# bcgsc/abyss

Hardware: AMD Instinct MI355X
Metric: Mk-mers/s inserted+extended (abyss-bloom-dbg, k=64); unitig bit-exact (higher is better)
Workload: dtype u64

## Files before the change

abyss_amd/_lib.py:

```python
from __future__ import annotations

import ctypes as C
import os

from . import build

ABG_OK = 0
ABG_EINVAL, ABG_ENODEV, ABG_ENOMEM, ABG_EINTERNAL, ABG_EAGAIN = -1, -2, -3, -4, -5


class Params(C.Structure):
    _fields_ = [
        ("k", C.c_uint32), ("num_hashes", C.c_uint32), ("min_cov", C.c_uint32), ("trim", C.c_uint32),
        ("bloom_bytes", C.c_uint64), ("counters", C.c_uint64), ("spaced_seed", C.c_char_p),
        ("device", C.c_int32), ("verbose", C.c_int32), ("insert_batch_kmers", C.c_uint64),
        ("claim_log2", C.c_uint32), ("walk_slots", C.c_uint32), ("wtab_log2", C.c_uint32),
        ("cascade_levels", C.c_uint32), ("slice_filter", C.c_uint32), ("reserved_", C.c_uint32 * 5),
    ]


class Counters(C.Structure):
    _fields_ = [(n, C.c_uint64) for n in
                ("solid_reads", "visited_reads", "reads_processed", "bases_assembled", "next_contig_id")]


class Contig(C.Structure):
    _fields_ = [
        ("contig_id", C.c_uint64), ("read_index", C.c_uint64), ("seq", C.c_char_p),
        ("length", C.c_uint32), ("coverage", C.c_uint32), ("redundant", C.c_int32),
        ("left_ext", C.c_uint32), ("right_ext", C.c_uint32), ("left_code", C.c_int32),
        ("right_code", C.c_int32), ("seed_pos", C.c_uint32),
    ]


class Stats(C.Structure):
    _fields_ = [(n, C.c_uint64) for n in
                ("insert_rounds", "walk_rounds", "candidates", "walked", "rewalked", "commit_breaks",
                 "commit_rounds", "generated", "bulk_calls", "bulk_steps", "lin_steps", "guide_slots", "chain_steps", "batch_cuts", "overflows", "memo_hits", "memo_adds", "tiled_ops", "tiled_pending", "tile_overflows", "cls_covered_reads", "archive_bases", "cls_decided_reads", "counter_bytes_held",
                 "commit_rounds_incremental", "commit_dirty_records", "commit_first_chunk_decided")]


CONTIG_CB = C.CFUNCTYPE(None, C.c_void_p, C.POINTER(Contig))
TEXT_CB = C.CFUNCTYPE(None, C.c_void_p, C.POINTER(C.c_char), C.c_uint64)

_lib = None


def symbols():
    return [
        "abg_params_init", "abg_create", "abg_destroy", "abg_last_error", "abg_reset", "abg_filter_size",
        "abg_load_seqs", "abg_load_seqs_v", "abg_keep_reads", "abg_assemble_kept", "abg_load_packed", "abg_counting_stats", "abg_counters_export",
        "abg_counters_import", "abg_visited_export", "abg_visited_import", "abg_assemble_seqs", "abg_assemble_seqs_v",
        "abg_assemble_packed", "abg_cascade_export", "abg_get_counters", "abg_set_counters", "abg_hash_seq",
        "abg_contains_seq",
        "abg_attach_comm", "abg_share_reads", "abg_rccl_unique_id", "abg_rccl_comm_create", "abg_rccl_comm_destroy",
        "abg_dev_copy", "abg_dev_alloc", "abg_dev_free", "abg_output_graph_seqs",
        "abg_profile_enable", "abg_profile_reset", "abg_profile_get", "abg_get_stats",
        "abg_overlap_create", "abg_overlap_destroy", "abg_overlap_last_error", "abg_overlap_join", "abg_overlap_edges",
        "abg_overlap_profile", "abg_overlap_profile_get",
        "abg_rr_create", "abg_rr_destroy", "abg_rr_last_error", "abg_rr_bytes", "abg_rr_clear", "abg_rr_insert_seqs",
        "abg_rr_contains_seqs", "abg_rr_popcount", "abg_rr_export", "abg_rr_sync", "abg_rr_profile", "abg_rr_profile_get",
        "abg_kn_create", "abg_kn_destroy", "abg_kn_last_error", "abg_kn_import", "abg_kn_export", "abg_kn_insert_seqs",
        "abg_kn_contains_seqs", "abg_kn_popcount", "abg_kn_hash_seq", "abg_kn_sync", "abg_kn_profile", "abg_kn_profile_get",
        "abg_fm_create", "abg_fm_destroy", "abg_fm_last_error", "abg_fm_build", "abg_fm_size", "abg_fm_export", "abg_fm_map_seqs",
        "abg_fm_sync", "abg_fm_tune", "abg_fm_profile", "abg_fm_profile_get",
    ]


def load(path: str | None = None):
    global _lib
    if _lib is not None:
        return _lib
# ... 99 lines not shown
```

abyss_amd/csrc/abg_core.h:

```cpp
#pragma once

#include <stdint.h>
#include <stddef.h>

#if defined(__HIPCC__)
#include <hip/hip_runtime.h>
#define ABG_HD __host__ __device__ __forceinline__
#define ABG_HDN __host__ __device__
#define ABG_HDX __host__ __device__ __attribute__((noinline))
#else
#define ABG_HD inline
#define ABG_HDN
#define ABG_HDX
#endif

namespace abg {

constexpr int MAX_NW = 6;
constexpr int MAX_HASHES = 32;
constexpr unsigned FP_TRIM = 5;

enum Dir : int { FORWARD = 0, REVERSE = 1 };
enum Sense : int { SENSE = 0, ANTISENSE = 1 };

// ... 1141 lines not shown
{
	if (!coop) return atomic_min_u32(p, v);
	uint32_t r = 0;
	if (__lane_id() == 0) r = atomic_min_u32(p, v);
	return (uint32_t)__builtin_amdgcn_readfirstlane((int)r);
}
ABG_HD uint32_t wu_atomic_add_u32(uint32_t* p, uint32_t v, bool coop)
{
	if (!coop) return atomic_add_u32(p, v);
	uint32_t r = 0;
	if (__lane_id() == 0) r = atomic_add_u32(p, v);
	return (uint32_t)__builtin_amdgcn_readfirstlane((int)r);
}
ABG_HD uint64_t wu_atomic_add_u64(uint64_t* p, uint64_t v, bool coop)
{
	if (!coop) return atomic_add_u64(p, v);
	uint64_t r = 0;
	if (__lane_id() == 0) r = atomic_add_u64(p, v);
	return ((uint64_t)(uint32_t)__builtin_amdgcn_readfirstlane((int)(r >> 32)) << 32) |
	       (uint32_t)__builtin_amdgcn_readfirstlane((int)(uint32_t)r);
}
ABG_HD void wu_st_coherent(uint64_t* p, uint64_t v, bool coop)
{
	if (!coop || __lane_id() == 0) st_coherent(p, v);
}
ABG_HD void wu_st_u32(uint32_t* p, uint32_t v, bool coop)
{
	if (!coop || __lane_id() == 0) *p = v;
}
ABG_HD void wu_st_u8(uint8_t* p, uint8_t v, bool coop)
{
	if (!coop || __lane_id() == 0) *p = v;
}
#else
ABG_HD void wu_st_coherent(uint64_t* p, uint64_t v, bool) { st_coherent(p, v); }
ABG_HD void wu_st_u32(uint32_t* p, uint32_t v, bool) { *p = v; }
ABG_HD void wu_st_u8(uint8_t* p, uint8_t v, bool) { *p = v; }
ABG_HD uint64_t wu_cas_u64(uint64_t* p, uint64_t e, uint64_t v, bool) { return cas_u64(p, e, v); }
ABG_HD uint32_t wu_atomic_min_u32(uint32_t* p, uint32_t v, bool) { return atomic_min_u32(p, v); }
ABG_HD uint32_t wu_atomic_add_u32(uint32_t* p, uint32_t v, bool) { return atomic_add_u32(p, v); }
ABG_HD uint64_t wu_atomic_add_u64(uint64_t* p, uint64_t v, bool) { return atomic_add_u64(p, v); }
#endif

struct Guide {
	const uint64_t* tab;
	uint64_t mask;
	const uint32_t* words;
	uint64_t nwords;
	uint8_t* seen;
};
constexpr unsigned SV_VALID = 0x80u, SV_SIMPLE = 0x01u;
constexpr uint32_t GUIDE_MAX_NK = 256;
ABG_HD uint64_t guide_slot(uint64_t hm, uint64_t mask)
{
	uint64_t x = hm * 0x9E3779B97F4A7C15ULL;
	x ^= x >> 29;
	return x & mask;
}
ABG_HD uint32_t guide_tag(uint64_t hm) { return (uint32_t)(hm >> 56); }
ABG_HD uint64_t guide_pack(uint64_t woff, uint32_t pos, uint32_t nk, uint32_t tag)
{
	return (1ULL << 63) | ((uint64_t)(tag & 0xFFu) << 55) | ((uint64_t)(nk - 1) << 47) | ((uint64_t)pos << 39) | woff;
}
constexpr uint64_t GUIDE_MAX_WOFF = (1ULL << 39) - 1;
constexpr uint32_t BULK_LANES = 64, BULK_MIN = 4;
struct BulkScratch {
	VKey key[BULK_LANES];
	uint8_t good[BULK_LANES];
	uint8_t fbase[BULK_LANES];
	uint32_t dup[2 * BULK_LANES];
	uint32_t dupstop;
	uint32_t full;
	uint64_t hw[MAX_NW], hfh, hrh, hdf, hdr;
	struct Chain { uint64_t w[MAX_NW], fh, rh, df, dr; uint32_t depth, state; } chain[4];
};
enum { CB_ACTIVE = 0,
       CB_TRUE = 1,
       CB_NOT_CHAIN = 2,
       CB_NONE = 3,
       CB_FALSE = 4 };
enum { WSTAT_BULK_CALLS = 0, WSTAT_BULK_STEPS, WSTAT_LIN_STEPS, WSTAT_CHAIN_STEPS, WSTAT_MEMO_HITS, WSTAT_MEMO_ADDS,
       WSTAT_OVF_POOL, WSTAT_OVF_RECS,
       WSTAT_CLS_COVERED,
       WSTAT_CLS_DECIDED,
       WSTAT_N = 16 };

struct SuccMemo {
	uint64_t* k0;
	uint64_t* k1;
	uint64_t* val;
	uint64_t mask;
};
constexpr uint64_t MEMO_EMPTY = ~0ULL;
constexpr unsigned MEMO_PROBES = 8;
ABG_HD uint64_t memo_slot(const SuccMemo& m, uint64_t fh, uint64_t rh, int dir)
{
	uint64_t x = (fh ^ (rh * 0x9E3779B97F4A7C15ULL)) + (uint64_t)dir;
	x ^= x >> 31; x *= 0xD6E8FEB86659FD93ULL; x ^= x >> 29;
	return x & m.mask;
}
ABG_HD int memo_find(const SuccMemo& m, uint64_t fh, uint64_t rh, int dir)
{
	if (fh == MEMO_EMPTY || rh == MEMO_EMPTY) return -1;
	uint64_t s = memo_slot(m, fh, rh, dir);
	for (unsigned i = 0; i < MEMO_PROBES; i++, s = (s + 1) & m.mask) {
		const uint64_t a = ld_coherent(&m.k0[s]);
		if (a == MEMO_EMPTY) return -1;
		if (a != fh) continue;
		const uint64_t v = ld_coherent(&m.val[s]);
		if (!(v >> 63) || (int)((v >> 8) & 1u) != dir) continue;
		if (ld_coherent(&m.k1[s]) != rh) continue;
		return (int)(v & 0xFFu);
	}
	return -1;
}
ABG_HD void memo_add(const SuccMemo& m, uint64_t fh, uint64_t rh, int dir, unsigned code, unsigned base, bool coop)
{
// ... 895 lines not shown
```

abyss_amd/csrc/abg_engine.h:

```cpp
#pragma once
#include "abg_walk.h"

#include <algorithm>
#include <chrono>
#include <cstdio>
#include <cstdlib>
#include <cstring>
#include <functional>
#include <future>
#include <string>
#include <type_traits>
#include <vector>

namespace abg {

struct Failure { int code; std::string msg; };
constexpr int FAIL_INVAL = -1, FAIL_NOMEM = -3, FAIL_INTERNAL = -4;
[[noreturn]] inline void fail_now(int code, const std::string& msg) { throw Failure{ code, msg }; }
inline std::string strf(const char* fmt, unsigned long long a = 0, unsigned long long b = 0)
{
	char buf[256];
	snprintf(buf, sizeof buf, fmt, a, b);
	return buf;
}
// ... 17 lines not shown
	bool cosettle = true;
	uint32_t cosettle_passes = 6;
	uint32_t cosettle_log2 = 24;
	uint32_t walk_slots = 4096;
	uint32_t tb_cap = 512;
	uint32_t buf_cap = 1u << 16;
	uint64_t pool_cap = 1ull << 28;
	uint32_t rec_cap = 1u << 22;
	uint32_t wtab_log2 = 26;
	uint32_t wtab_log2_max = 31;
	uint32_t cend_log2 = 20;
	uint64_t p2_first_batch = 65536;
	uint64_t p2_max_batch = 1ull << 22;
	uint32_t p2_growth = 2;
	uint32_t p2_crowded = 1u << 18;
	uint32_t p2_starved_growth = 2;
	uint32_t p2_starved = 6144;
	uint32_t slice_filter = 0;
	bool solid_plane = true;
	uint32_t classify_slots = 65536;
	uint32_t cls_both_max_mb = 1024;
	bool cls_both = true;
	bool prefetch_classify = true;
	uint32_t memo_log2 = 0;
	bool memo = true;
	uint32_t p2_max_candidates = 1u << 18;
	uint32_t t_tags = 1024;
	uint32_t commit_incremental = 1;
	uint32_t commit_dirty_max = 4096;
	uint32_t commit_dirty_log2 = 26;
	uint32_t guide_stride = 4;
	uint32_t guide_log2_max = 31;
	bool guide_seen = true;
	bool link_duplicates = true;
	bool par_commit = true;
	bool overlap_bins = true;
	bool overlap_purity = true;
	uint32_t dist_hash_all_ranks = 2;
	uint32_t dist_route_min_ranks = 4;
	uint64_t keep_insert_scratch_bytes = 16ull << 30;
	uint64_t par_commit_max_bytes = 16ull << 30;
	int verbose = 0;
};

struct Counters {
	uint64_t solid_reads = 0, visited_reads = 0, reads_processed = 0, bases_assembled = 0,
	         contig_id = 0;
};

struct BaseCodes {
	uint8_t t[256];
	BaseCodes()
	{
		for (int i = 0; i < 256; i++) t[i] = 0xFF;
		t['A'] = t['a'] = 0; t['C'] = t['c'] = 1; t['G'] = t['g'] = 2; t['T'] = t['t'] = 3;
	}
};
template <class T>
struct NoInitAlloc : std::allocator<T> {
	template <class U> struct rebind { using other = NoInitAlloc<U>; };
	template <class U, class... A> void construct(U* p, A&&... a)
	{
		if constexpr (sizeof...(A) == 0) ::new ((void*)p) U; else ::new ((void*)p) U(std::forward<A>(a)...);
	}
};
struct HostBatch {
// ... 3183 lines not shown
			if (guide_tab_) be_.free(guide_tab_);
			guide_tab_ = (uint64_t*)be_.try_alloc(8ull << log2);
			guide_log2_ = log2;
			if (!guide_tab_) { if (cfg_.verbose) fprintf(stderr, "abyss_amd: no memory for the walkers' guide table, walking step by step\n"); return; }
		}
		be_.memset(guide_tab_, 0, 8ull << log2);
		guide_.mask = (1ull << log2) - 1; guide_.words = b.words; guide_.nwords = nwords;
		dispatch_nw([&](auto nw) {
			FGuideBuild<decltype(nw)::value> f{ p2_, b, cnt2_, guide_tab_, guide_.mask, cfg_.guide_stride, sampled };
			be_.launch_wave((sampled + GUIDE_READS_PER_ITEM - 1) / GUIDE_READS_PER_ITEM, f, "guide_build");
		});
		guide_.tab = guide_tab_;
		guide_slots_ = guide_.mask + 1;
		if (cfg_.guide_seen) {
			const uint64_t need = nwords * 16, total = be_.device_mem_bytes();
			if (guide_seen_ && guide_seen_bytes_ < need) { be_.free(guide_seen_); guide_seen_ = nullptr; }
			if (!guide_seen_ && (!total || need <= total / 24)) { guide_seen_ = (uint8_t*)be_.try_alloc(need); guide_seen_bytes_ = need; }
			if (guide_seen_) { be_.memset(guide_seen_, 0, need); guide_.seen = guide_seen_; }
		}
	}
	uint64_t next_batch_size() const
	{
		if (last_candidates_ > cfg_.p2_crowded) return std::max<uint64_t>(p2_batch_ / 2, 1024);
		if (last_candidates_ < cfg_.p2_starved) return std::min<uint64_t>(p2_batch_ * cfg_.p2_starved_growth, 8 * cfg_.p2_max_batch);
		return std::min<uint64_t>(p2_batch_ * cfg_.p2_growth, cfg_.p2_max_batch);
	}
	void clear_wstats()
	{
		be_.memset(wstats_, 0, WSTAT_N * 8);
	}
	struct Stats { uint64_t rounds = 0, walked = 0, rewalked = 0, candidates = 0, breaks = 0, insert_rounds = 0, commit_rounds = 0, generated = 0;
	               uint64_t bulk_calls = 0, bulk_steps = 0, lin_steps = 0, guide_slots = 0, chain_steps = 0, batch_cuts = 0, overflows = 0, memo_hits = 0, memo_adds = 0;
	               uint64_t tiled_ops = 0, tiled_pending = 0, tile_overflows = 0, cls_covered_reads = 0, archive_bases = 0, cls_decided_reads = 0;
	               uint64_t commit_rounds_incremental = 0, commit_dirty_records = 0, commit_first_chunk_decided = 0; };
	Stats stats()
	{
		Stats s = stats_;
		if (wstats_) {
			uint64_t v[WSTAT_N];
			be_.d2h(v, wstats_, sizeof v);
			s.bulk_calls = v[WSTAT_BULK_CALLS]; s.bulk_steps = v[WSTAT_BULK_STEPS]; s.lin_steps = v[WSTAT_LIN_STEPS]; s.chain_steps = v[WSTAT_CHAIN_STEPS];
			s.memo_hits = v[WSTAT_MEMO_HITS]; s.memo_adds = v[WSTAT_MEMO_ADDS];
			s.cls_covered_reads = v[WSTAT_CLS_COVERED]; s.cls_decided_reads = v[WSTAT_CLS_DECIDED];
		}
		if (arc_.seq && arc_valid_) { uint64_t u = 0; be_.d2h(&u, arc_.used, 8); s.archive_bases = std::min(u, arc_.cap) - ARC_HEAD; }
		s.guide_slots = guide_slots_;
		return s;
	}

  private:
	BE& be_;
	Config cfg_;
	Params p_;
	uint64_t m_ = 0, vis_bytes_ = 0;
	uint8_t* cnt_ = nullptr;
	uint8_t* vis_ = nullptr;
	CommitState* cstate_ = nullptr;
	uint64_t* scal_ = nullptr;
	Cascade casc_{ nullptr, 0, 0 };
	MaskTab* mask_d_ = nullptr;
	std::chrono::steady_clock::time_point dbg_t0_;
	uint32_t* T_ = nullptr;
	uint32_t t_tag_ = 0;
	uint64_t* Tk_ = nullptr; uint32_t* Tv_ = nullptr; uint32_t Tlog2_ = 0;
	uint64_t T_entries_ = 0;
	uint32_t* pcA_ = nullptr; uint64_t pcA_bits_ = 0; uint32_t pcA_shift_ = 0;
	bool t_hashed() const { return t_force_hashed_ || m_ * 4ull > cfg_.par_commit_max_bytes; }
	bool t_force_hashed_ = false;
	bool use_par_commit()
	{
		if (!cfg_.par_commit || t_failed_) return false;
		if (t_hashed()) return true;
		if (!T_) {
			T_ = (uint32_t*)be_.try_alloc(m_ * 4ull);
			t_tag_ = 0;
			if (!T_ && sliced_) {
// ... 746 lines not shown
		walk_ready_ = false;
	}
	void grow_walk_resources()
	{
		free_walk_scratch();
		walk_tb_cap_ *= 4;
		walk_buf_cap_ *= 8;
		if (walk_buf_cap_ > (1u << 28) || wtab_log2_ > 31) {
			fail_now(FAIL_INTERNAL, "a unitig exceeds the walker limits");
		}
		while ((uint64_t)wslots_ * walk_buf_cap_ > (8ull << 30) && wslots_ > 64) wslots_ /= 2;
		alloc_walk_scratch();
		free_tab(wtab_);
		wtab_log2_++;
		alloc_tab(wtab_, wtab_log2_);
		be_.free(pool_); be_.free(kh_);
		pool_cap_ *= 2;
		pool_ = (uint8_t*)be_.alloc(pool_cap_);
		kh_ = (uint64_t*)be_.alloc(pool_cap_ * 8);
		if (cfg_.verbose)
			fprintf(stderr, "abyss_amd: walker resources grown: %u frames, %u bases, 2^%u table, %llu pool\n",
			    walk_tb_cap_, walk_buf_cap_, wtab_log2_, (unsigned long long)pool_cap_);
	}

	template <int NW>
	WalkEnv<NW> make_env(const Batch& b, uint32_t* cand_d, uint32_t* status_d, uint32_t* first_d)
	{
		WalkEnv<NW> e;
		e.p = p2_; e.cnt = cnt2_; e.batch = b; e.cand_read = cand_d; e.status = status_d; e.first_rec = first_d;
		e.tab = wtab_; e.owner_base = 0;
		e.tb_pool = (TBFrame<NW>*)tb_pool_;
		e.tbk_pool = tbk_pool_;
		e.tb_cap = walk_tb_cap_;
		e.fast = nullptr; e.fast_bytes = 0; e.dbg = dbg_; e.coop = false;
		e.la_pool = la_pool_;
		e.guide = guide_; e.bulk_pool = bulk_pool_; e.wstats = wstats_; e.memo = memo_; e.mcache = nullptr;
		e.lbuf_pool = lbuf_; e.rbuf_pool = rbuf_; e.buf_cap = walk_buf_cap_;
		e.pool = pool_; e.pool_cap = pool_cap_; e.pool_used = pool_used_;
		e.recs = recs_; e.rec_cap = rec_cap_; e.rec_used = rec_used_;
		return e;
	}

	template <int NW>
	uint32_t commit(const Batch& b, uint32_t* cand_d, uint32_t* status_d, uint32_t* first_d,
	    uint8_t* result_d, const uint64_t* rkoff_d, uint32_t c_begin, uint32_t c_end)
	{
		{
			uint32_t nrec = 0, nord = 0;
			be_.d2h(&nrec, rec_used_, 4);
			be_.d2h(&nord, order_n_, 4);
			uint64_t need = cend_count_ + 2ull * (std::min(nrec, rec_cap_) - std::min(nord, rec_cap_));
			while (need * 2 > cend_.mask + 1) grow_cend();
		}
		CommitState cs;
		cs.counters = counters_;
		cs.break_at = c_begin; cs.pad_ = 0; cs.cend_count = cend_count_;
		be_.h2d(cstate_, &cs, sizeof cs);
		{
			FPreCommit<NW> f{ p_, b, cand_d, status_d, first_d, recs_, vis_, kh_, rkh_, rkoff_d, read_flag_, c_begin, 0, ~0ULL, nullptr, nullptr, nullptr };
			be_.launch_wave(c_end - c_begin, f, "precommit");
			FPreCommitCopies fc{ status_d, first_d, recs_, read_flag_, c_begin, p_.k };
			be_.launch(c_end - c_begin, fc, "precommit");
		}
		CommitEnv<NW> e;
		e.read_flag = read_flag_;
		e.p = p_; e.b = b; e.vis32 = (uint32_t*)vis_; e.both32 = (uint32_t*)both_;
		e.cand_read = cand_d; e.status = status_d; e.first_rec = first_d;
// ... 696 lines not shown
```

abyss_amd/csrc/abg_host.h:

```cpp
#pragma once
#include "abg_engine.h"
#include "../../include/abyss_amd.h"

#include <cctype>
#include <cmath>
#include <map>
#include <string>
#include <atomic>
#include <chrono>
#include <future>
#include <memory>
#include <thread>

namespace abg {
static_assert(FAIL_NOMEM == ABG_ENOMEM && FAIL_INTERNAL == ABG_EINTERNAL, "Failure codes are the C ABI's");


struct FContainsSolid {
	Params p; const uint64_t* h0; const uint8_t* cnt; uint8_t* out;
	ABG_HD void operator()(uint64_t t, uint32_t) const { out[t] = solid_contains(p, cnt, h0[t]) ? 1 : 0; }
};
struct FExpand {
	Params p; const uint64_t* h0; uint64_t* out;
	ABG_HD void operator()(uint64_t t, uint32_t) const
// ... 46 lines not shown
		cfg.verbose = p.verbose;
		if (p.insert_batch_kmers) cfg.insert_batch_kmers = p.insert_batch_kmers;
		if (p.claim_log2) cfg.claim_log2 = p.claim_log2;
		if (p.walk_slots) cfg.walk_slots = p.walk_slots;
		if (p.wtab_log2) cfg.wtab_log2 = p.wtab_log2;
		if (const char* e = getenv("ABG_CLAIM_LOG2")) cfg.claim_log2 = (uint32_t)atoi(e);
		if (const char* e = getenv("ABG_INSERT_BATCH")) cfg.insert_batch_kmers = strtoull(e, 0, 10);
		if (const char* e = getenv("ABG_WALK_SLOTS")) cfg.walk_slots = (uint32_t)atoi(e);
		if (const char* e = getenv("ABG_WTAB_LOG2")) cfg.wtab_log2 = (uint32_t)atoi(e);
		if (const char* e = getenv("ABG_WTAB_LOG2_MAX")) cfg.wtab_log2_max = (uint32_t)std::max<int>(atoi(e), (int)cfg.wtab_log2);
		if (const char* e = getenv("ABG_POOL_CAP")) cfg.pool_cap = std::max<uint64_t>(1024, strtoull(e, 0, 10));
		if (const char* e = getenv("ABG_REC_CAP")) cfg.rec_cap = (uint32_t)std::max(16, atoi(e));
		if (const char* e = getenv("ABG_P2_FIRST_BATCH")) cfg.p2_first_batch = strtoull(e, 0, 10);
		if (const char* e = getenv("ABG_P2_MAX_BATCH")) cfg.p2_max_batch = strtoull(e, 0, 10);
		if (const char* e = getenv("ABG_PAR_COMMIT")) cfg.par_commit = atoi(e) != 0;
		if (const char* e = getenv("ABG_T_TAGS")) cfg.t_tags = (uint32_t)std::max(2, atoi(e));
		if (const char* e = getenv("ABG_COMMIT_INCREMENTAL")) cfg.commit_incremental = (uint32_t)std::min(2, std::max(0, atoi(e)));
		if (const char* e = getenv("ABG_COMMIT_DIRTY_MAX")) cfg.commit_dirty_max = (uint32_t)std::max(0, atoi(e));
		if (const char* e = getenv("ABG_COMMIT_DIRTY_LOG2")) cfg.commit_dirty_log2 = (uint32_t)std::min(34, std::max(10, atoi(e)));
		if (const char* e = getenv("ABG_PAR_COMMIT_MAX_GB")) cfg.par_commit_max_bytes = strtoull(e, 0, 10) << 30;
		if (const char* e = getenv("ABG_COMPACT_THRESHOLD")) cfg.compact_threshold = strtoull(e, 0, 10);
		if (const char* e = getenv("ABG_TILED")) cfg.tiled_insert = atoi(e) != 0;
		if (const char* e = getenv("ABG_DIST_ROUTE_MIN")) cfg.dist_route_min_ranks = (uint32_t)atoi(e);
		if (const char* e = getenv("ABG_BENIGN")) cfg.benign_sharers = atoi(e) != 0;
		if (const char* e = getenv("ABG_CLS_ARCHIVE")) cfg.cls_archive = atoi(e) != 0;
		if (const char* e = getenv("ABG_CLS_DEBUG_SKIP")) cfg.cls_debug_skip = (uint32_t)atoi(e);
		if (const char* e = getenv("ABG_CLS_ARCHIVE_MAX_MB")) cfg.cls_archive_max_mb = (uint32_t)std::max(0, atoi(e));
		if (const char* e = getenv("ABG_SORTED_OVERFLOW")) cfg.sorted_overflow = atoi(e) != 0;
		if (const char* e = getenv("ABG_COSETTLE")) cfg.cosettle = atoi(e) != 0;
		if (const char* e = getenv("ABG_CLS_BOTH")) cfg.cls_both = atoi(e) != 0;
		if (const char* e = getenv("ABG_CLS_BOTH_MAX_MB")) cfg.cls_both_max_mb = (uint32_t)std::max(0, atoi(e));
		if (const char* e = getenv("ABG_COSETTLE_PASSES")) cfg.cosettle_passes = (uint32_t)std::max(1, atoi(e));
		if (const char* e = getenv("ABG_COSETTLE_LOG2")) cfg.cosettle_log2 = (uint32_t)std::min(25, std::max(5, atoi(e)));
		if (const char* e = getenv("ABG_LINK_DUPS")) cfg.link_duplicates = atoi(e) != 0;
		if (const char* e = getenv("ABG_OVERLAP_PURITY")) cfg.overlap_purity = atoi(e) != 0;
		if (const char* e = getenv("ABG_OVERLAP_BINS")) cfg.overlap_bins = atoi(e) != 0;
		if (const char* e = getenv("ABG_PREFETCH")) cfg.prefetch_classify = atoi(e) != 0;
		if (const char* e = getenv("ABG_ASYNC_LOAD")) cfg.async_load = atoi(e) != 0;
		if (const char* e = getenv("ABG_CLS_SLOTS")) cfg.classify_slots = (uint32_t)std::max(64, atoi(e));
		if (const char* e = getenv("ABG_SOLID_PLANE")) cfg.solid_plane = atoi(e) != 0;
		if (const char* e = getenv("ABG_MEMO")) cfg.memo = atoi(e) != 0;
		if (const char* e = getenv("ABG_P2_MAX_CANDIDATES")) cfg.p2_max_candidates = (uint32_t)std::max(1, atoi(e));
		if (const char* e = getenv("ABG_P2_STARVED_GROWTH")) cfg.p2_starved_growth = (uint32_t)std::max(2, atoi(e));
		if (const char* e = getenv("ABG_P2_STARVED")) cfg.p2_starved = (uint32_t)atoi(e);
		if (const char* e = getenv("ABG_P2_GROWTH")) cfg.p2_growth = (uint32_t)std::max(2, atoi(e));
		if (const char* e = getenv("ABG_DRAIN_THRESHOLD")) cfg.drain_threshold = (uint32_t)strtoul(e, 0, 10);
		if (const char* e = getenv("ABG_GUIDE_STRIDE")) cfg.guide_stride = (uint32_t)strtoul(e, 0, 10);
		if (const char* e = getenv("ABG_GUIDE_SEEN")) cfg.guide_seen = atoi(e) != 0;
		if (const char* e = getenv("ABG_GUIDE_LOG2_MAX")) cfg.guide_log2_max = (uint32_t)std::min(36, std::max(10, atoi(e)));
		if (!be.ok()) return fail(ABG_ENODEV, be.why());
		eng = new Engine<BE>(be, cfg);
		return ABG_OK;
	}

	int load_seqs(const char* seqs, const uint64_t* off, uint64_t n) { return load_seqs_v(1, &seqs, &off, &n); }
	int load_seqs_v(uint32_t nchunks, const char* const* seqs_v, const uint64_t* const* off_v, const uint64_t* n_v)
	{
		const uint32_t k = cfg.k;
		const double t_call = std::chrono::duration<double>(std::chrono::steady_clock::now().time_since_epoch()).count();
		const uint32_t max_piece = (uint32_t)std::min<uint64_t>(1u << 20, cfg.insert_batch_kmers + k - 1);
		struct Part { uint32_t c; uint64_t a, b; };
		std::vector<Part> plan;
		std::vector<uint64_t> base(nchunks + 1, 0);
		for (uint32_t c = 0; c < nchunks; c++) {
			base[c + 1] = base[c] + n_v[c];
			if (!n_v[c]) continue;
// ... 736 lines not shown
```

abyss_amd/csrc/abg_kernels.hip:

```cpp
#include <hip/hip_runtime.h>
#include <hip/hip_ext.h>
#include <hipcub/hipcub.hpp>
#include <rccl/rccl.h>
#include <dlfcn.h>
#include <unistd.h>

#include "abg_host.h"
#include "abg_overlap.h"

#include <chrono>
#include <map>
#include <mutex>

namespace {

template <class F>
__global__ void __launch_bounds__(256) k_foreach(F f, uint64_t n)
{
	uint64_t i = (uint64_t)blockIdx.x * blockDim.x + threadIdx.x;
	const uint64_t stride = (uint64_t)gridDim.x * blockDim.x;
	const uint32_t slot = (uint32_t)i;
	for (; i < n; i += stride) f(i, slot);
}
#ifndef ABG_CLS_WAVES
// ... 1074 lines not shown
}
int abg_profile_get(abg_ctx* ctx, const char* name, double* total_ms, uint64_t* launches)
{
	if (!ctx || !name) return ABG_EINVAL;
	return guarded(ctx, [&]() -> int {
		ctx->s.be.prof_drain();
		auto it = ctx->s.be.prof.find(name);
		double ms = 0;
		uint64_t n = 0;
		if (it != ctx->s.be.prof.end()) { ms = it->second.ms; n = it->second.launches; }
		if (total_ms) *total_ms = ms;
		if (launches) *launches = n;
		return ABG_OK;
	});
}
int abg_get_stats(const abg_ctx* ctx, abg_stats* out)
{
	if (!ctx || !out) return ABG_EINVAL;
	return guarded((abg_ctx*)ctx, [&]() -> int {
		auto s = ctx->s.eng->stats();
		out->insert_rounds = s.insert_rounds;
		out->walk_rounds = s.rounds;
		out->candidates = s.candidates;
		out->walked = s.walked;
		out->rewalked = s.rewalked;
		out->commit_breaks = s.breaks; out->commit_rounds = s.commit_rounds; out->generated = s.generated;
		out->bulk_calls = s.bulk_calls; out->bulk_steps = s.bulk_steps; out->lin_steps = s.lin_steps; out->guide_slots = s.guide_slots; out->chain_steps = s.chain_steps; out->batch_cuts = s.batch_cuts; out->overflows = s.overflows;
		out->memo_hits = s.memo_hits; out->memo_adds = s.memo_adds;
		out->tiled_ops = s.tiled_ops; out->tiled_pending = s.tiled_pending; out->tile_overflows = s.tile_overflows;
		out->cls_covered_reads = s.cls_covered_reads; out->archive_bases = s.archive_bases; out->cls_decided_reads = s.cls_decided_reads;
		out->counter_bytes_held = ctx->s.eng->counter_bytes_held();
		out->commit_rounds_incremental = s.commit_rounds_incremental; out->commit_dirty_records = s.commit_dirty_records;
		out->commit_first_chunk_decided = s.commit_first_chunk_decided;
		return ABG_OK;
	});
}

}
struct abg_overlap {
	HipBackend be;
	abg::OverlapJoin<HipBackend> join;
	std::string error;
	explicit abg_overlap(int dev) : be(dev), join(be) {}
};
namespace {
std::string g_overlap_create_error;
template <class F>
int guarded_ov(abg_overlap* o, F&& body)
{
	try {
		return body();
	} catch (const abg::Failure& f) {
		o->error = f.msg;
		return f.code;
	} catch (const std::bad_alloc&) {
		o->error = "host memory exhausted";
		return ABG_ENOMEM;
	} catch (const std::exception& e) {
		o->error = e.what();
		return ABG_EINTERNAL;
	}
}
}
extern "C" {
int abg_overlap_create(int device, abg_overlap** out)
{
// ... 58 lines not shown
```

abyss_amd/csrc/abg_walk.h:

```cpp
#pragma once
#include "abg_core.h"

namespace abg {

struct Batch {
	const uint32_t* words;
	const uint64_t* woff;
	const uint32_t* len;
	const uint64_t* koff;
	uint64_t n;
};
ABG_HD unsigned batch_base(const Batch& b, uint64_t r, uint32_t i)
{
	uint32_t w = b.words[b.woff[r] + (i >> 4)];
	return (w >> (2 * (i & 15))) & 3u;
}
template <int NW>
ABG_HD Kmer<NW> batch_kmer(const Batch& b, uint64_t r, uint32_t pos, unsigned k)
{
	return window_kmer<NW>(b.words, b.woff[r], pos, k);
}
ABG_HD uint64_t find_seq(const uint64_t* koff, uint64_t n, uint64_t t)
{
	uint64_t lo = 0, hi = n;
// ... 74 lines not shown
	uint32_t cand;
	uint32_t next;
	uint32_t seed_pos;
	uint32_t left_ext, right_ext;
	uint8_t left_code, right_code;
	uint8_t redundant;
	uint8_t pre_redundant;
	uint32_t coverage;
	uint64_t contig_id;
	uint32_t time;
	uint32_t ins;
	uint32_t ins_prev;
	uint32_t dup_of;
	uint64_t fp;
};
constexpr uint32_t REC_END = 0xFFFFFFFFu;

template <int NW>
struct WalkEnv {
	Params p;
	const uint8_t* cnt;
	Batch batch;
	const uint32_t* cand_read;
	uint32_t* status;
	uint32_t* first_rec;
	WalkTab tab;
	uint32_t owner_base;
	TBFrame<NW>* tb_pool; VKey* tbk_pool; uint32_t tb_cap;
	void* fast; uint32_t fast_bytes;
	VKey* la_pool;
	uint8_t* lbuf_pool; uint8_t* rbuf_pool; uint32_t buf_cap;
	uint64_t* dbg;
	bool coop;
	Guide guide;
	SuccMemo memo;
	MaskCache* mcache;
	BulkScratch* bulk_pool;
	uint64_t* wstats;
	uint8_t* pool; uint64_t pool_cap; uint64_t* pool_used;
	ContigRec* recs; uint32_t rec_cap; uint32_t* rec_used;
};

template <int NW>
struct WalkState {
	Vtx<NW> seed;
	uint8_t* lbuf; uint8_t* rbuf;
	uint32_t nl, nr;
	Vtx<NW> head;
	VKey prev_key;
	uint32_t ext;
	int32_t ins;
	BulkScratch* bulk;
	uint32_t bulk_skip;
	uint32_t bulk_overflow;
	uint32_t n_bulk_calls, n_bulk_steps, n_lin_steps;
	uint32_t n_bulk_tries;
	uint64_t t_bx[6];
	uint64_t t_seed, t_ext, t_mat;
	uint64_t t_bulk, t_lin, t_post;
	uint64_t t_bp[4];
};
template <int NW>
ABG_HD unsigned ws_base(const Params& p, const WalkState<NW>& w, uint32_t j)
{
	if (j < w.nl) return w.lbuf[w.nl - 1 - j];
	j -= w.nl;
// ... 588 lines not shown
	sc.overflow = 0;
	sc.dbg_search = 0; sc.dbg_calls = 0; sc.dbg_nodes = 0; sc.dbg_chain = 0; sc.dbg_on = e.dbg ? 1u : 0u; sc.n_chain_steps = 0; sc.dbg_la = 0; sc.dbg_la_calls = 0; sc.dbg_mask = 0; sc.dbg_mask_n = 0; sc.dbg_memo = 0;
	sc.coop = e.coop;
	sc.la_visited = e.la_pool + (uint64_t)slot * LA_MAX_VISITED;
}

#if defined(__HIP_DEVICE_COMPILE__)
template <int NW>
ABG_HDN uint32_t next_unassembled(const WalkEnv<NW>& e, uint64_t r, uint32_t it, uint32_t nk, uint32_t owner)
{
	const Params& p = e.p;
	const uint32_t* __restrict__ words = e.batch.words;
	const uint64_t woff = e.batch.woff[r];
	const uint32_t lane = lane_id();
	for (uint32_t base = it; base < nk; base += 64u) {
		const uint32_t n = nk - base < 64u ? nk - base : 64u;
		uint64_t fh, rh;
		stretch_hashes_wave<NW>(words, woff, base, n, p.k, fh, rh);
		bool missing = false;
		if (lane < n) {
			const Kmer<NW> s = window_kmer<NW>(words, woff, base + lane, p.k);
			uint64_t df = 0, dr = 0;
			if constexpr (MASKED_BUILD<NW>) masked_terms(p, s, df, dr);
			const uint64_t fs = wt_find(e.tab, wt_key(kmer_ident(p, s, fh, rh, df, dr)), owner);
			missing = fs == WT_EMPTY || (uint32_t)ld_coherent(&e.tab.meta[fs]) == WT_TOMB;
		}
		const uint64_t b = wave_ballot(missing);
		if (b) return base + (uint32_t)__builtin_ctzll(b);
	}
	return nk;
}
#endif
template <int NW>
ABG_HDN void walk_read(WalkEnv<NW>& e, uint32_t c, uint32_t slot)
{
	const Params& p = e.p;
	const unsigned k = p.k;
	SearchScratch<NW>* scp; WalkState<NW>* wp;
	walker_scratch(e, slot, scp, wp);
	SearchScratch<NW>& sc = *scp;
	WalkState<NW>& w = *wp;
#if defined(__HIP_DEVICE_COMPILE__)
	const uint64_t t_start = wall_clock64();
#else
	const uint64_t t_start = 0;
#endif
	uint64_t total_steps = 0;

	w.lbuf = e.lbuf_pool + (uint64_t)slot * e.buf_cap;
	w.rbuf = e.rbuf_pool + (uint64_t)slot * e.buf_cap;

	const uint64_t r = e.cand_read[c];
	const uint32_t L = e.batch.len[r];
	const uint32_t nk = L - k + 1;
	const uint32_t owner = e.owner_base + c;
	uint32_t first = REC_END, last = REC_END, contig = 0;
	uint32_t abort_status = 0;

	Vtx<NW> cur;
	cur.s = batch_kmer<NW>(e.batch, r, 0, k);
	vtx_rehash(p, cur);
	uint64_t ts0 = dbg_clock(e.dbg);
	for (uint32_t it = 0; it < nk; it++) {
		VKey ckey;
#if defined(__HIP_DEVICE_COMPILE__)
		if (sc.coop) {
			it = next_unassembled(e, r, it, nk, owner);
			if (it >= nk) break;
			cur.s = window_kmer<NW>(e.batch.words, e.batch.woff[r], it, k);
			vtx_rehash(p, cur);
			ckey = vtx_key(p, cur);
		} else
#endif
		{
			if (it > 0) vtx_shift(p, cur, SENSE, (uint32_t)batch_base(e.batch, r, it + k - 1));
			ckey = vtx_key(p, cur);
			uint64_t fs = wt_find(e.tab, ckey, owner);
			if (fs != WT_EMPTY && (uint32_t)ld_coherent(&e.tab.meta[fs]) != WT_TOMB) continue;
		}
		if (e.dbg) w.t_seed += dbg_clock(e.dbg) - ts0;
		const uint64_t te0 = dbg_clock(e.dbg);

		w.seed = cur; w.nl = 0; w.nr = 0;
		int ins = wt_insert(e.tab, ckey, owner, contig, sc.coop);
		if (ins == WT_FULL) { abort_status = WS_OVERFLOW; break; }
		bool seed_earlier = (ins == WT_EARLIER);
		bool left_earlier = seed_earlier, right_earlier = seed_earlier;
		uint32_t lext = 0, rext = 0;
		int lcode = walk_extend(e, w, REVERSE, owner, contig, sc, &lext, &abort_status, &left_earlier);
		if (lcode < 0) break;
		int rcode = walk_extend(e, w, FORWARD, owner, contig, sc, &rext, &abort_status, &right_earlier);
		if (rcode < 0) break;
		uint32_t n = w.nl + 1 + w.nr;
		total_steps += n;
		const uint64_t tp0 = dbg_clock(e.dbg);
		if (e.dbg) w.t_ext += tp0 - te0;

		const bool tip = is_tip(n, lcode, rcode, p.trim);
		if (!tip) {
			uint64_t need = (uint64_t)n + k - 1 + 2;
			uint64_t off = wu_atomic_add_u64(e.pool_used, need, sc.coop);
			if (off + need > e.pool_cap) {
				wu_atomic_add_u64(&e.wstats[WSTAT_OVF_POOL], 1, sc.coop);
				abort_status = WS_OVERFLOW; break;
			}
			uint8_t* S = e.pool + off + 1;
			uint64_t slen = (uint64_t)n + k - 1;
			for (uint64_t j = sc.coop ? lane_id() : 0u; j < slen; j += sc.coop ? 64u : 1u) S[j] = (uint8_t)ws_base(p, w, (uint32_t)j);
			wave_sync();
			int64_t lo = 0, hi = (int64_t)n;
			Vtx<NW> popped[2]; bool popped_earlier[2]; int npopped = 0;
// ... 51 lines not shown
				wu_atomic_add_u64(&e.wstats[WSTAT_OVF_RECS], 1, sc.coop);
				abort_status = WS_OVERFLOW; break;
			}
			ContigRec& rec = e.recs[ri];
			rec.seq_off = off + 1 + (uint64_t)lo;
			rec.len = (uint32_t)(hi - lo) + k - 1;
			rec.cand = c; rec.next = REC_END; rec.seed_pos = it;
			rec.left_ext = lext; rec.right_ext = rext;
			rec.left_code = (uint8_t)lcode; rec.right_code = (uint8_t)rcode;
			rec.redundant = 0; rec.pre_redundant = 0; rec.coverage = 0; rec.contig_id = ~0ULL;
			rec.ins_prev = 0; rec.dup_of = REC_END; rec.fp = 0;
			if (last == REC_END) first = ri; else e.recs[last].next = ri;
			last = ri;
			if (npopped) {
				Vtx<NW> nf = pool_vertex<NW>(p, S, lo, sc.coop), nb = pool_vertex<NW>(p, S, hi - 1, sc.coop);
				if (pushed_side < 0) nf = pushed;
				if (pushed_side > 0) nb = pushed;
				for (int q = 0; q < npopped; q++) {
					if (popped_earlier[q]) continue;
					if (hi > lo && (vtx_equal(p, popped[q], nf) || vtx_equal(p, popped[q], nb))) continue;
					uint64_t s = wt_find(e.tab, vtx_key(p, popped[q]), owner);
					if (s != WT_EMPTY) wu_st_coherent(&e.tab.meta[s], ((uint64_t)owner << 32) | WT_TOMB, sc.coop);
				}
			}
			if (p.mask && hi > lo && (uint64_t)(hi - lo) < k) {
				const MaskTab& m = *p.mask;
				const uint32_t np = (uint32_t)(hi - lo);
				uint8_t* C = S + lo;
				for (uint32_t col = np; col + 1 < k; col++) {
					uint32_t j0 = col - np + 1, j1 = col + 1;
					if (m.ones_prefix[j1] == m.ones_prefix[j0]) C[col] = 4;
				}
			}
		}
		contig++;
		if (e.dbg) { ts0 = dbg_clock(e.dbg); w.t_post += ts0 - tp0; }
	}
	e.first_rec[c] = first;
	e.status[c] = abort_status ? abort_status : (uint32_t)WS_COMPLETE;
	if (e.wstats) {
		wu_atomic_add_u64(&e.wstats[WSTAT_BULK_CALLS], w.n_bulk_calls, sc.coop);
		wu_atomic_add_u64(&e.wstats[WSTAT_BULK_STEPS], w.n_bulk_steps, sc.coop);
		wu_atomic_add_u64(&e.wstats[WSTAT_LIN_STEPS], w.n_lin_steps, sc.coop);
		wu_atomic_add_u64(&e.wstats[WSTAT_CHAIN_STEPS], sc.n_chain_steps, sc.coop);
		wu_atomic_add_u64(&e.wstats[WSTAT_MEMO_HITS], sc.n_memo_hits, sc.coop);
		wu_atomic_add_u64(&e.wstats[WSTAT_MEMO_ADDS], sc.n_memo_adds, sc.coop);
	}
	if (e.dbg) {
#if defined(__HIP_DEVICE_COMPILE__)
		const uint64_t t_end = wall_clock64();
#else
		const uint64_t t_end = 0;
#endif
		uint64_t* d = e.dbg + (uint64_t)c * WALK_DBG_N;
		d[0] = t_end - t_start; d[1] = total_steps; d[2] = sc.dbg_search; d[3] = sc.dbg_calls;
		d[4] = sc.dbg_nodes; d[5] = w.t_bulk; d[6] = contig; d[7] = w.t_post;
		d[8] = w.t_lin; d[9] = w.n_bulk_tries; d[10] = w.n_bulk_calls; d[11] = w.n_bulk_steps; d[12] = sc.dbg_chain;
		d[13] = sc.dbg_la; d[14] = sc.dbg_la_calls; d[15] = w.t_bp[1]; d[16] = sc.dbg_mask; d[17] = sc.dbg_mask_n; d[18] = sc.dbg_memo;
		d[19] = w.t_seed + (dbg_clock(e.dbg) - ts0); d[20] = w.t_ext; d[21] = w.t_mat;
		for (int q = 0; q < 6; q++) d[22 + q] = w.t_bx[q];
	}
}

ABG_HD unsigned code_rank(unsigned c) { return c == 4 ? 3u : (c == 3 ? 4u : c); }
ABG_HD unsigned code_comp(unsigned c) { return c == 4 ? 4u : 3u - c; }
ABG_HDN VKey canonical_end_key(const Params& p, const uint8_t* seq)
// ... 29 lines not shown
```

include/abyss_amd.h:

```cpp
#ifndef ABYSS_AMD_H
#define ABYSS_AMD_H 1

#include <stddef.h>
#include <stdint.h>

#ifdef __cplusplus
extern "C" {
#endif

#define ABG_OK 0
#define ABG_EINVAL (-1)
#define ABG_ENODEV (-2)
#define ABG_ENOMEM (-3)
#define ABG_EINTERNAL (-4)
#define ABG_EAGAIN (-5)

#define ABG_MAX_KMER 192
#define ABG_MAX_HASHES 32

enum abg_read_result {
	ABG_RR_UNINITIALIZED = 0,
	ABG_RR_SHORTER_THAN_K,
	ABG_RR_NON_ACGT,
	ABG_RR_BLUNT_END,
// ... 120 lines not shown

int abg_dev_copy(abg_ctx* ctx, void* dst, const void* src, uint64_t n, int32_t kind);
int abg_dev_alloc(abg_ctx* ctx, uint64_t bytes, void** out);
int abg_dev_free(abg_ctx* ctx, void* ptr);

typedef void (*abg_text_cb)(void* user, const char* text, uint64_t len);
int abg_output_graph_seqs(abg_ctx* ctx, const char* seqs, const uint64_t* offsets, uint64_t n,
    abg_text_cb cb, void* user, uint64_t* nodes, uint64_t* edges);

int abg_profile_enable(abg_ctx* ctx, int on);
int abg_profile_reset(abg_ctx* ctx);
int abg_profile_get(abg_ctx* ctx, const char* name, double* total_ms, uint64_t* launches);
typedef struct abg_stats {
	uint64_t insert_rounds, walk_rounds, candidates, walked, rewalked, commit_breaks;
	uint64_t commit_rounds;
	uint64_t generated;
	uint64_t bulk_calls, bulk_steps;
	uint64_t lin_steps;
	uint64_t guide_slots;
	uint64_t chain_steps;
	uint64_t batch_cuts;
	uint64_t overflows;
	uint64_t memo_hits, memo_adds;
	uint64_t tiled_ops;
	uint64_t tiled_pending;
	uint64_t tile_overflows;
	uint64_t cls_covered_reads;
	uint64_t archive_bases;
	uint64_t cls_decided_reads;
	uint64_t counter_bytes_held;
	uint64_t commit_rounds_incremental;
	uint64_t commit_dirty_records;
	uint64_t commit_first_chunk_decided;
} abg_stats;
int abg_get_stats(const abg_ctx* ctx, abg_stats* out);

typedef struct abg_overlap abg_overlap;
int abg_overlap_create(int device, abg_overlap** out);
void abg_overlap_destroy(abg_overlap* o);
const char* abg_overlap_last_error(const abg_overlap* o);
int abg_overlap_join(abg_overlap* o, uint32_t overlap, uint64_t n_contigs, const uint64_t* head_keys,
    const uint64_t* tail_keys, int strand_specific, uint64_t* n_edges);
int abg_overlap_edges(abg_overlap* o, uint64_t* offsets, uint32_t* targets);
int abg_overlap_profile(abg_overlap* o, int on);
int abg_overlap_profile_get(abg_overlap* o, const char* name, double* total_ms, uint64_t* launches);

typedef struct abg_rr abg_rr;
int abg_rr_create(int device, uint64_t bytes, uint32_t hash_num, uint32_t r, abg_rr** out);
void abg_rr_destroy(abg_rr* f);
const char* abg_rr_last_error(const abg_rr* f);
int abg_rr_bytes(const abg_rr* f, uint64_t* bytes);
int abg_rr_clear(abg_rr* f);
int abg_rr_insert_seqs(abg_rr* f, const char* seqs, const uint64_t* offsets, uint64_t n, uint32_t max_bases,
    const uint32_t* lengths, uint32_t n_lengths, uint64_t* n_inserted);
int abg_rr_contains_seqs(abg_rr* f, const char* seqs, const uint64_t* offsets, uint64_t n, uint32_t* found);
int abg_rr_popcount(abg_rr* f, uint64_t* bits_set);
int abg_rr_export(abg_rr* f, uint8_t* host_out);
int abg_rr_sync(abg_rr* f);
int abg_rr_profile(abg_rr* f, int on);
int abg_rr_profile_get(abg_rr* f, const char* name, double* total_ms, uint64_t* launches);


typedef struct abg_kn abg_kn;
int abg_kn_create(int device, uint64_t full_bits, uint32_t levels, uint32_t k, uint64_t seed, uint64_t start, uint64_t end,
    abg_kn** out);
void abg_kn_destroy(abg_kn* f);
// ... 33 lines not shown
```

Before: 1603.

## Skip seed lookups for read k-mers already covered by the walked contig

After a contig is walked from a read, the new code compares the read's bases after the seed against the contig's right extension. It advances the seed iterator past every k-mer that matches, so those positions skip the walk-table lookup or next_unassembled scan. It also skips the visited check for the first k-mer of each read and adds wavefront-ballot matching for the cooperative path. Two counters are added to the stats to measure seed scans and matched skips. The risk is a change in bit-exactness if the match logic disagrees with the table state, plus some extra atomic counter traffic.

```diff
diff --git a/abyss_amd/_lib.py b/abyss_amd/_lib.py
--- a/abyss_amd/_lib.py
+++ b/abyss_amd/_lib.py
@@ -37,7 +37,8 @@
     _fields_ = [(n, C.c_uint64) for n in
                 ("insert_rounds", "walk_rounds", "candidates", "walked", "rewalked", "commit_breaks",
                  "commit_rounds", "generated", "bulk_calls", "bulk_steps", "lin_steps", "guide_slots", "chain_steps", "batch_cuts", "overflows", "memo_hits", "memo_adds", "tiled_ops", "tiled_pending", "tile_overflows", "cls_covered_reads", "archive_bases", "cls_decided_reads", "counter_bytes_held",
-                 "commit_rounds_incremental", "commit_dirty_records", "commit_first_chunk_decided")]
+                 "commit_rounds_incremental", "commit_dirty_records", "commit_first_chunk_decided",
+                 "walk_seed_scans", "walk_seed_matched")]
 
 
 CONTIG_CB = C.CFUNCTYPE(None, C.c_void_p, C.POINTER(Contig))
diff --git a/abyss_amd/csrc/abg_core.h b/abyss_amd/csrc/abg_core.h
--- a/abyss_amd/csrc/abg_core.h
+++ b/abyss_amd/csrc/abg_core.h
@@ -1197,7 +1197,12 @@
 {
 	if (!coop || __lane_id() == 0) *p = v;
 }
+ABG_HD void wu_count(uint64_t* p, uint64_t v, bool coop)
+{
+	if (!coop || __lane_id() == 0) atomic_add_u64(p, v);
+}
 #else
+ABG_HD void wu_count(uint64_t* p, uint64_t v, bool) { *p += v; }
 ABG_HD void wu_st_coherent(uint64_t* p, uint64_t v, bool) { st_coherent(p, v); }
 ABG_HD void wu_st_u32(uint32_t* p, uint32_t v, bool) { *p = v; }
 ABG_HD void wu_st_u8(uint8_t* p, uint8_t v, bool) { *p = v; }
@@ -1248,6 +1253,8 @@
        WSTAT_OVF_POOL, WSTAT_OVF_RECS,
        WSTAT_CLS_COVERED,
        WSTAT_CLS_DECIDED,
+       WSTAT_SEED_SCANS,
+       WSTAT_SEED_MATCHED,
        WSTAT_N = 16 };
 
 struct SuccMemo {
diff --git a/abyss_amd/csrc/abg_engine.h b/abyss_amd/csrc/abg_engine.h
--- a/abyss_amd/csrc/abg_engine.h
+++ b/abyss_amd/csrc/abg_engine.h
@@ -73,6 +73,7 @@
 	uint32_t guide_stride = 4;
 	uint32_t guide_log2_max = 31;
 	bool guide_seen = true;
+	bool walk_read_match = true;
 	bool link_duplicates = true;
 	bool par_commit = true;
 	bool overlap_bins = true;
@@ -3322,7 +3323,8 @@
 	struct Stats { uint64_t rounds = 0, walked = 0, rewalked = 0, candidates = 0, breaks = 0, insert_rounds = 0, commit_rounds = 0, generated = 0;
 	               uint64_t bulk_calls = 0, bulk_steps = 0, lin_steps = 0, guide_slots = 0, chain_steps = 0, batch_cuts = 0, overflows = 0, memo_hits = 0, memo_adds = 0;
 	               uint64_t tiled_ops = 0, tiled_pending = 0, tile_overflows = 0, cls_covered_reads = 0, archive_bases = 0, cls_decided_reads = 0;
-	               uint64_t commit_rounds_incremental = 0, commit_dirty_records = 0, commit_first_chunk_decided = 0; };
+	               uint64_t commit_rounds_incremental = 0, commit_dirty_records = 0, commit_first_chunk_decided = 0;
+	               uint64_t walk_seed_scans = 0, walk_seed_matched = 0; };
 	Stats stats()
 	{
 		Stats s = stats_;
@@ -3332,6 +3334,7 @@
 			s.bulk_calls = v[WSTAT_BULK_CALLS]; s.bulk_steps = v[WSTAT_BULK_STEPS]; s.lin_steps = v[WSTAT_LIN_STEPS]; s.chain_steps = v[WSTAT_CHAIN_STEPS];
 			s.memo_hits = v[WSTAT_MEMO_HITS]; s.memo_adds = v[WSTAT_MEMO_ADDS];
 			s.cls_covered_reads = v[WSTAT_CLS_COVERED]; s.cls_decided_reads = v[WSTAT_CLS_DECIDED];
+			if (!dist()) { s.walk_seed_scans = v[WSTAT_SEED_SCANS]; s.walk_seed_matched = v[WSTAT_SEED_MATCHED]; }
 		}
 		if (arc_.seq && arc_valid_) { uint64_t u = 0; be_.d2h(&u, arc_.used, 8); s.archive_bases = std::min(u, arc_.cap) - ARC_HEAD; }
 		s.guide_slots = guide_slots_;
@@ -4144,7 +4147,7 @@
 		e.tb_pool = (TBFrame<NW>*)tb_pool_;
 		e.tbk_pool = tbk_pool_;
 		e.tb_cap = walk_tb_cap_;
-		e.fast = nullptr; e.fast_bytes = 0; e.dbg = dbg_; e.coop = false;
+		e.fast = nullptr; e.fast_bytes = 0; e.dbg = dbg_; e.coop = false; e.read_match = cfg_.walk_read_match;
 		e.la_pool = la_pool_;
 		e.guide = guide_; e.bulk_pool = bulk_pool_; e.wstats = wstats_; e.memo = memo_; e.mcache = nullptr;
 		e.lbuf_pool = lbuf_; e.rbuf_pool = rbuf_; e.buf_cap = walk_buf_cap_;
diff --git a/abyss_amd/csrc/abg_host.h b/abyss_amd/csrc/abg_host.h
--- a/abyss_amd/csrc/abg_host.h
+++ b/abyss_amd/csrc/abg_host.h
@@ -102,6 +102,7 @@
 		if (const char* e = getenv("ABG_CLS_BOTH_MAX_MB")) cfg.cls_both_max_mb = (uint32_t)std::max(0, atoi(e));
 		if (const char* e = getenv("ABG_COSETTLE_PASSES")) cfg.cosettle_passes = (uint32_t)std::max(1, atoi(e));
 		if (const char* e = getenv("ABG_COSETTLE_LOG2")) cfg.cosettle_log2 = (uint32_t)std::min(25, std::max(5, atoi(e)));
+		if (const char* e = getenv("ABG_WALK_READ_MATCH")) cfg.walk_read_match = atoi(e) != 0;
 		if (const char* e = getenv("ABG_LINK_DUPS")) cfg.link_duplicates = atoi(e) != 0;
 		if (const char* e = getenv("ABG_OVERLAP_PURITY")) cfg.overlap_purity = atoi(e) != 0;
 		if (const char* e = getenv("ABG_OVERLAP_BINS")) cfg.overlap_bins = atoi(e) != 0;
diff --git a/abyss_amd/csrc/abg_kernels.hip b/abyss_amd/csrc/abg_kernels.hip
--- a/abyss_amd/csrc/abg_kernels.hip
+++ b/abyss_amd/csrc/abg_kernels.hip
@@ -1130,6 +1130,7 @@
 		out->counter_bytes_held = ctx->s.eng->counter_bytes_held();
 		out->commit_rounds_incremental = s.commit_rounds_incremental; out->commit_dirty_records = s.commit_dirty_records;
 		out->commit_first_chunk_decided = s.commit_first_chunk_decided;
+		out->walk_seed_scans = s.walk_seed_scans; out->walk_seed_matched = s.walk_seed_matched;
 		return ABG_OK;
 	});
 }
diff --git a/abyss_amd/csrc/abg_walk.h b/abyss_amd/csrc/abg_walk.h
--- a/abyss_amd/csrc/abg_walk.h
+++ b/abyss_amd/csrc/abg_walk.h
@@ -130,6 +130,7 @@
 	uint8_t* lbuf_pool; uint8_t* rbuf_pool; uint32_t buf_cap;
 	uint64_t* dbg;
 	bool coop;
+	bool read_match;
 	Guide guide;
 	SuccMemo memo;
 	MaskCache* mcache;
@@ -784,6 +785,35 @@
 }
 #endif
 template <int NW>
+ABG_HDN uint32_t seed_matched(const WalkEnv<NW>& e, uint64_t r, uint32_t it, uint32_t nk, const uint8_t* S, uint32_t nl,
+    uint32_t kept_hi, bool coop)
+{
+	if (kept_hi <= nl + 1 || it + 1 >= nk) return 0;
+	uint32_t lim = kept_hi - 1 - nl;
+	if (lim > nk - 1 - it) lim = nk - 1 - it;
+	const uint32_t rb = it + e.p.k;
+	const uint8_t* sp = S + nl + e.p.k;
+#if defined(__HIP_DEVICE_COMPILE__)
+	if (coop) {
+		const uint32_t* __restrict__ words = e.batch.words;
+		const uint64_t woff = e.batch.woff[r];
+		const uint32_t lane = lane_id();
+		for (uint32_t base = 0; base < lim; base += 64u) {
+			const uint32_t j = base + lane < lim ? base + lane : lim - 1u;
+			const uint32_t w = words[woff + ((rb + j) >> 4)];
+			const unsigned s = sp[j];
+			const uint64_t b = wave_ballot(((w >> (2 * ((rb + j) & 15u))) & 3u) != s);
+			if (b) return base + (uint32_t)__builtin_ctzll(b);
+		}
+		return lim;
+	}
+#endif
+	(void)coop;
+	uint32_t j = 0;
+	while (j < lim && batch_base(e.batch, r, rb + j) == (unsigned)sp[j]) j++;
+	return j;
+}
+template <int NW>
 ABG_HDN void walk_read(WalkEnv<NW>& e, uint32_t c, uint32_t slot)
 {
 	const Params& p = e.p;
@@ -813,12 +843,17 @@
 	cur.s = batch_kmer<NW>(e.batch, r, 0, k);
 	vtx_rehash(p, cur);
 	uint64_t ts0 = dbg_clock(e.dbg);
+	constexpr bool READ_MATCH = !MASKED_BUILD<NW>;
+	bool scanning = false;
 	for (uint32_t it = 0; it < nk; it++) {
 		VKey ckey;
 #if defined(__HIP_DEVICE_COMPILE__)
 		if (sc.coop) {
-			it = next_unassembled(e, r, it, nk, owner);
-			if (it >= nk) break;
+			if (!(READ_MATCH && e.read_match && it == 0)) {
+				if constexpr (READ_MATCH) wu_count(&e.wstats[WSTAT_SEED_SCANS], 1, true);
+				it = next_unassembled(e, r, it, nk, owner);
+				if (it >= nk) break;
+			}
 			cur.s = window_kmer<NW>(e.batch.words, e.batch.woff[r], it, k);
 			vtx_rehash(p, cur);
 			ckey = vtx_key(p, cur);
@@ -827,8 +862,12 @@
 		{
 			if (it > 0) vtx_shift(p, cur, SENSE, (uint32_t)batch_base(e.batch, r, it + k - 1));
 			ckey = vtx_key(p, cur);
-			uint64_t fs = wt_find(e.tab, ckey, owner);
-			if (fs != WT_EMPTY && (uint32_t)ld_coherent(&e.tab.meta[fs]) != WT_TOMB) continue;
+			if (!(READ_MATCH && e.read_match && it == 0)) {
+				if (READ_MATCH && !scanning) { wu_count(&e.wstats[WSTAT_SEED_SCANS], 1, false); scanning = true; }
+				uint64_t fs = wt_find(e.tab, ckey, owner);
+				if (fs != WT_EMPTY && (uint32_t)ld_coherent(&e.tab.meta[fs]) != WT_TOMB) continue;
+			}
+			scanning = false;
 		}
 		if (e.dbg) w.t_seed += dbg_clock(e.dbg) - ts0;
 		const uint64_t te0 = dbg_clock(e.dbg);
@@ -946,6 +985,15 @@
 					if (m.ones_prefix[j1] == m.ones_prefix[j0]) C[col] = 4;
 				}
 			}
+			if constexpr (READ_MATCH) if (e.read_match) {
+				const uint32_t kept_hi = (uint32_t)(hi < (int64_t)n ? hi : (int64_t)n);
+				const uint32_t m = seed_matched(e, r, it, nk, S, w.nl, kept_hi, sc.coop);
+				if (m) {
+					wu_count(&e.wstats[WSTAT_SEED_MATCHED], m, sc.coop);
+					if (!sc.coop) for (uint32_t q = 1; q <= m; q++) vtx_shift(p, cur, SENSE, (uint32_t)batch_base(e.batch, r, it + q + k - 1));
+					it += m;
+				}
+			}
 		}
 		contig++;
 		if (e.dbg) { ts0 = dbg_clock(e.dbg); w.t_post += ts0 - tp0; }
diff --git a/include/abyss_amd.h b/include/abyss_amd.h
--- a/include/abyss_amd.h
+++ b/include/abyss_amd.h
@@ -176,6 +176,8 @@
 	uint64_t commit_rounds_incremental;
 	uint64_t commit_dirty_records;
 	uint64_t commit_first_chunk_decided;
+	uint64_t walk_seed_scans;
+	uint64_t walk_seed_matched;
 } abg_stats;
 int abg_get_stats(const abg_ctx* ctx, abg_stats* out);
 
```

After: 1618, median of 6. No clear change (+0.9%).
